# Gyeeta/gyeeta

Measured on NVIDIA H100. Metric: events/sec aggregated, higher is better.
Workload: dtype u64

## Files before the change

### gyeeta_b200/csrc/gysk_device.cuh

```cuda
#pragma once

#include <cstdint>
#include <cuda_runtime.h>

namespace gysk {

struct HistCell { unsigned long long count; long long sum; };
static constexpr int HIST_CELLS = 16;
static constexpr int HIST_MAX_CELL = 15;

struct alignas(16) TblEntry { unsigned long long key; uint32_t slot1; uint32_t pad; };
static constexpr uint32_t SLOT_INVALID = 0xFFFFFFFFu;

struct Centroid { double mean; unsigned long long weight; };
static constexpr int TD_CAP = 256;

struct alignas(16) Bin { unsigned long long cw; unsigned long long us; };
static constexpr int NBINS = 848;
static constexpr int BIN_CNT_BITS = 27;
static constexpr unsigned long long BIN_CNT_MASK = (1ull << BIN_CNT_BITS) - 1;
static constexpr int HOT_ROW_BINS = 1024, HOT_ROW_WORDS = 2 * HOT_ROW_BINS;
static_assert(NBINS <= HOT_ROW_BINS, "a row holds every bin");
__host__ __device__ __forceinline__ uint32_t hot_word(uint32_t bin) { return ((bin & 31u) << 5) | (bin >> 5); }

struct alignas(8) SlotAux { unsigned long long act_cur, act_last, err_cur, err_last; uint32_t rtt_cur, rtt_last; };

struct alignas(16) SlotBatch { uint32_t minv, maxv, touched, hot; };
struct alignas(8) SlotState { uint8_t state, issue, issue_bits, high_bits; uint32_t nconn_active; };

struct TdHead { unsigned long long total; double minv, maxv; uint32_t n; uint32_t pad; };

struct IdTable
{
	TblEntry	*ent;
	uint32_t	mask;
	uint32_t	max_slots;
	uint32_t	*count;
	unsigned long long *slot_id;
	uint32_t	*slot_host;
	int32_t		*free_n;
	uint32_t	*free_slots;
	unsigned long long *insert_fail;
};
static constexpr unsigned long long KEY_TOMBSTONE = ~0ull;

enum { CTR_IN = 0, CTR_DROPPED, CTR_RESP, CTR_TCP, CTR_TASK, CTR_FOREIGN, CTR_NKEYS, CTR_INSERT_FAIL, CTR_NTOUCHED ,
	CTR_NLONG , CTR_NEVICT, CTR_EVICTED_TOTAL,
	CTR_NHOT , CTR_NHOT_NEXT , CTR_NWINDOW ,
	CTR_NHOSTS , CTR_MAX };

static constexpr uint32_t JHASH_GOLDEN = 0x9e3779b9u;
static constexpr uint32_t GY_SEED = 0xceedfeadu;
static constexpr uint32_t FLOW_SEED_A = GY_SEED;
static constexpr uint32_t FLOW_SEED_B = GY_SEED ^ 0x5bd1e995u;

__host__ __device__ __forceinline__ uint32_t jhash_2words(uint32_t a, uint32_t b, uint32_t initval)
{
	uint32_t c = initval;

	a += JHASH_GOLDEN; b += JHASH_GOLDEN;
	a -= b; a -= c; a ^= (c >> 13);
	b -= c; b -= a; b ^= (a << 8);
	c -= a; c -= b; c ^= (b >> 13);
	a -= b; a -= c; a ^= (c >> 12);
	b -= c; b -= a; b ^= (a << 16);
	c -= a; c -= b; c ^= (b >> 5);
	a -= b; a -= c; a ^= (c >> 3);
	b -= c; b -= a; b ^= (a << 10);
	c -= a; c -= b; c ^= (b >> 15);
	return c;
}

__host__ __device__ __forceinline__ uint32_t uint64_hash(unsigned long long key)
{
	return jhash_2words((uint32_t)(key & 0xFFFFFFFFu), (uint32_t)(key >> 32), GY_SEED);
}

__host__ __device__ __forceinline__ uint32_t table_hash(unsigned long long key)
{
	return (uint32_t)((key * 0x9E3779B97F4A7C15ull) >> 32);
}

__host__ __device__ __forceinline__ void flow_hashes(unsigned long long key, uint32_t &h1, uint32_t &h2)
{
	const uint32_t lo = (uint32_t)key, hi = (uint32_t)(key >> 32);
	h1 = jhash_2words(lo, hi, FLOW_SEED_A);
	h2 = jhash_2words(lo, hi, FLOW_SEED_B);
}

__host__ __device__ __forceinline__ uint32_t cms_index2(uint32_t h1, uint32_t h2, uint32_t row, uint32_t wmask)
{
	return (h1 + row * (h2 | 1u)) & wmask;
}

__host__ __device__ __forceinline__ uint32_t cms_index(unsigned long long key, uint32_t row, uint32_t wmask)
{
	uint32_t h1, h2;
	flow_hashes(key, h1, h2);
	return cms_index2(h1, h2, row, wmask);
}

__host__ __device__ __forceinline__ unsigned long long cms_increment(uint32_t bytes)
{
	return 1ull | ((unsigned long long)(bytes >> 10) << 32);
}

__device__ __forceinline__ void hll_idx_rank2(uint32_t h1, uint32_t h2, uint32_t p, uint32_t &idx, uint32_t &rank)
{
	const unsigned long long h = ((unsigned long long)h2 << 32) | h1;
	const unsigned long long w = h << p;

	idx = (uint32_t)(h >> (64 - p));
	rank = w ? (uint32_t)__clzll((long long)w) + 1u : (64u - p + 1u);
}

static constexpr int TD_CODE_BITS = 10;
__host__ __device__ __forceinline__ uint32_t td_code(uint32_t v)
{
#ifdef __CUDA_ARCH__
	if (v < 32u) return v;
	const uint32_t sh = (31u - (uint32_t)__clz((int)v)) - 5u;
#else
	if (v < 32u) return v;
	const uint32_t sh = (31u - (uint32_t)__builtin_clz(v)) - 5u;
#endif
	return ((sh + 1u) << 5) | ((v >> sh) & 31u);
}
__host__ __device__ __forceinline__ uint32_t td_code_lo(uint32_t c) { return c < 32u ? c : ((32u | (c & 31u)) << ((c >> 5) - 1u)); }
__host__ __device__ __forceinline__ uint32_t td_code_hi(uint32_t c) { return c < 32u ? c : (((32u | (c & 31u)) + 1u) << ((c >> 5) - 1u)) - 1u; }

// ... 178 lines not shown
```

### gyeeta_b200/csrc/gysk_kernels.cu

```cuda
#include "gysk_kernels.cuh"
#include "gysk_state.cuh"
#include "gysk_summary.cuh"

#include <cfloat>
#include <climits>
#include <cmath>
#include <algorithm>
#include <type_traits>
#include <cstdlib>
#include <cstring>

namespace gysk {

static constexpr int KEY_GROUP_SHIFT = 30;
static constexpr int KEY_SLOT_SHIFT = KEY_GROUP_SHIFT + TD_CODE_BITS;
__device__ __forceinline__ uint32_t key_usec(unsigned long long k) { return (uint32_t)k & 0x3FFFFFFFu; }
__device__ __forceinline__ uint32_t key_slot(unsigned long long k) { return (uint32_t)(k >> KEY_SLOT_SHIFT); }
__device__ __forceinline__ uint32_t key_bin(unsigned long long k) { return (uint32_t)(k >> KEY_GROUP_SHIFT) & ((1u << TD_CODE_BITS) - 1u); }

static constexpr int KEY_DIGIT_MAX = 8;
static constexpr int KEY_SLOT_BITS_MAX = 24;
static constexpr int KEY_PASSES_MAX = (TD_CODE_BITS + KEY_SLOT_BITS_MAX + KEY_DIGIT_MAX - 1) / KEY_DIGIT_MAX;
static_assert(KEY_PASSES_MAX <= OS_MAX_PASSES, "a RESP plan fits a SortPlan");
struct SortPlan { int np; int shift[OS_MAX_PASSES]; int bits[OS_MAX_PASSES]; };
// ... 823 lines not shown
	}
#pragma unroll
	for (int t = 0; t < LS_V; ++t) {
		const bool act = tail[t];
		if (!__any_sync(0xffffffffu, act)) continue;
		const uint32_t did = act ? pd[t] : (0x80000000u | (uint32_t)lane);
		const unsigned long long v = act ? ps[t] : 0ull;
		uint32_t cnt = act ? pc[t] : 0u, rem = act ? prem[t] : 0u;
		const uint32_t m = __match_any_sync(0xffffffffu, did);
		unsigned long long gsum = v;
		const uint32_t maxcnt = __reduce_max_sync(0xffffffffu, (uint32_t)__popc(m));
		uint32_t rest = m & ~(1u << lane);
		const uint32_t cnt0 = cnt, rem0 = rem;
		for (uint32_t u = 1; u < maxcnt; ++u) {
			const int src = rest ? (__ffs(rest) - 1) : lane;
			const unsigned long long ov = __shfl_sync(0xffffffffu, v, src);
			const uint32_t oc = __shfl_sync(0xffffffffu, cnt0, src), orr = __shfl_sync(0xffffffffu, rem0, src);
			if (rest) { gsum += ov; cnt += oc; rem += orr; rest &= rest - 1; }
		}
		if (act && (m & ((1u << lane) - 1u)) == 0) red_bin(did, (unsigned long long)cnt | ((unsigned long long)rem << BIN_CNT_BITS), gsum);
	}
}

__global__ void __launch_bounds__(256) long_sum_kernel(const unsigned long long *__restrict__ keys, const unsigned long long *__restrict__ d_n,
		const BatchSeg *__restrict__ segs, const unsigned long long *__restrict__ nlong, unsigned long long *__restrict__ rows)
{
	if (*nlong == 0) return;
	const uint64_t n = *d_n;
	const uint64_t nchunks = (n + 127) >> 7;
	const int lane = threadIdx.x & 31;
	const uint64_t gw = ((uint64_t)blockIdx.x * blockDim.x + threadIdx.x) >> 5, nwarps = ((uint64_t)gridDim.x * blockDim.x) >> 5;
	for (uint64_t c0 = gw * 32; c0 < nchunks; c0 += nwarps * 32) {
		const uint64_t c = c0 + lane;
		uint32_t sf = 0, sl = 0, rf = 0, rl = 0;
		if (c < nchunks) {
			const uint64_t f = c << 7, l = f + 127 < n ? f + 127 : n - 1;
			sf = key_slot(keys[f]); sl = key_slot(keys[l]);
			rf = segs[sf].row1; rl = segs[sl].row1;
		}
		for (uint32_t todo = __ballot_sync(0xffffffffu, (rf | rl) != 0); todo; todo &= todo - 1) {
			const int src = __ffs(todo) - 1;
			long_sum_chunk(keys, n, (c0 + (uint64_t)src) << 7, __shfl_sync(0xffffffffu, sf, src), __shfl_sync(0xffffffffu, rf, src),
					__shfl_sync(0xffffffffu, sl, src), __shfl_sync(0xffffffffu, rl, src), rows);
		}
	}
}

static constexpr int TD_WARPS = 3;
static constexpr int TD_SMEM_N = 540;

__global__ void __launch_bounds__(TD_WARPS * 32, TD_MERGE_CTAS_PER_SM) bins_merge_kernel(DevState st, const unsigned long long *__restrict__ keys,
		const uint32_t *__restrict__ touched, const unsigned long long *__restrict__ ntouched_p, const uint32_t *__restrict__ long_slot,
		const unsigned long long *__restrict__ nlong_p, unsigned long long *__restrict__ batch_rows, const BatchSeg *__restrict__ segs,
		Centroid *__restrict__ items_scratch , TdWorkBig *__restrict__ big_scratch , int exp)
{
	__shared__ TdWorkT<TD_SMEM_N> work[TD_WARPS];
	__shared__ uint32_t hcnt[TD_WARPS][16], hsum_lo[TD_WARPS][16], hsum_hi[TD_WARPS][16];
	__shared__ uint8_t bk_tab[NBINS / 8];
	const int lane = threadIdx.x & 31, wid = threadIdx.x >> 5;
	const uint32_t gw = blockIdx.x * TD_WARPS + wid, nwarps = gridDim.x * TD_WARPS;

	Centroid *items = items_scratch + (size_t)gw * NBINS;
	const uint32_t ntouched = (uint32_t)*ntouched_p, nlong = (uint32_t)*nlong_p;

	for (uint32_t g = threadIdx.x; g < (uint32_t)NBINS / 8; g += blockDim.x) {
		constexpr uint32_t thr[13] = {1, 10, 30, 60, 100, 150, 200, 300, 450, 700, 1000, 3000, 15000};
		auto bucket = [&](uint32_t bin) {
			uint32_t bk = bin >= 1u;
			for (int q = 2; q < 15; ++q) bk += bin >= td_code((thr[q - 2] + 1u) * 1000u) + (uint32_t)q;
			return bk;
		};
		const uint32_t b0 = bucket(g * 8);
		uint32_t off = 8;
		for (uint32_t o = 7; o >= 1; --o) if (bucket(g * 8 + o) != b0) off = o;
		bk_tab[g] = (uint8_t)(b0 | (off << 4));
	}
	__syncthreads();

	const uint32_t nhot = st.hot_rows ? (uint32_t)st.counters[CTR_NHOT] : 0u;
	const uint32_t nrow = nhot + nlong, total = nrow + ntouched;
	const uint32_t lt = (1u << lane) - 1u;
	auto slot_of = [&](uint32_t t) { return t < nhot ? st.hot_slot[t] : (t < nrow ? long_slot[t - nhot] : touched[t - nrow]); };
	uint32_t nslot = gw < total ? slot_of(gw) : 0u;
	for (uint32_t t = gw; t < total; t += nwarps) {
		const uint32_t slot = nslot;
		const bool has_next = t + nwarps < total;
		nslot = has_next ? slot_of(t + nwarps) : 0u;
		const SlotBatch sb = st.slot_batch[slot];
		BatchSeg seg {0u, 0u, 0u, 0u};
		if (t >= nrow) seg = segs[slot];
		uint2 nseg = make_uint2(0u, 0u);
		if (has_next) {
			prefetch_l2(st.td_cent + (size_t)nslot * TD_CAP + lane * (TD_CAP / 32));
			if (lane == 0) prefetch_l2(st.slot_batch + nslot);
			else if (lane == 1) prefetch_l2(st.td_head + nslot);
			if (t + nwarps >= nrow) { const BatchSeg ns = segs[nslot]; nseg = make_uint2(ns.key0, ns.end); }
		}
		if (t < nhot && sb.minv == 0xFFFFFFFFu) continue;
		if (lane < 16) { hcnt[wid][lane] = 0; hsum_lo[wid][lane] = 0; hsum_hi[wid][lane] = 0; }
		__syncwarp();
		const uint32_t na = st.td_head[slot].n;
		TdWorkT<TD_SMEM_N> &W = work[wid];
		auto take_bin = [&](uint32_t j, unsigned long long cw, unsigned long long us, uint32_t bin, bool staged) {
			const unsigned long long cnt = cw & BIN_CNT_MASK, rem = cw >> BIN_CNT_BITS;
			const double mean = __ddiv_rn((double)us, (double)cnt);
			if (staged) { W.src[na + j] = mean; W.nxt[j] = (uint16_t)cnt; }
			else { Centroid c; c.mean = mean; c.weight = cnt; items[j] = c; }
			const uint32_t e = bk_tab[bin >> 3], bk = (e & 15u) + ((bin & 7u) >= (e >> 4) ? 1u : 0u);
			atomicAdd(&hcnt[wid][bk], (uint32_t)cnt);
			const unsigned long long ms = (us - rem) / 1000ull;
			const uint32_t mlo = (uint32_t)ms, mhi = (uint32_t)(ms >> 32);
			const uint32_t old = atomicAdd(&hsum_lo[wid][bk], mlo);
			const uint32_t up = mhi + (old + mlo < old ? 1u : 0u);
			if (up) atomicAdd(&hsum_hi[wid][bk], up);
		};
		uint32_t nitems = 0, nsamples, binmax = 0;
		bool staged = false;
		if (t >= nrow) {
			nsamples = seg.end - seg.key0;
			constexpr int RAW_BIN_SHIFT = 54;
			static_assert(BIN_CNT_BITS + 10 + 14 <= RAW_BIN_SHIFT && LONG_SEG <= (1 << 14), "cw of a short segment's bin below the bin bits");
			const uint32_t room = (uint32_t)TD_SMEM_N - na;
			unsigned long long *raw_us = reinterpret_cast<unsigned long long *>(W.src + na), *raw_cw = W.pref;
			ulonglong2 *raw = reinterpret_cast<ulonglong2 *>(items);
			auto load8 = [&](uint32_t b0, unsigned long long (&k)[8]) {
				const uint32_t i0 = b0 + (uint32_t)lane * 8u;
				if (i0 >= seg.key0 && i0 + 8u <= seg.end) {
#pragma unroll
					for (int q = 0; q < 4; ++q) {
						const ulonglong2 v = *reinterpret_cast<const ulonglong2 *>(keys + i0 + 2 * q);
						k[2 * q] = v.x; k[2 * q + 1] = v.y;
					}
				}
				else {
#pragma unroll
					for (int u = 0; u < 8; ++u) k[u] = i0 + u >= seg.key0 && i0 + u < seg.end ? keys[i0 + u] : ~0ull;
				}
			};
			auto rem_of = [](uint32_t v) { return v - (v / 1000u) * 1000u; };
			uint32_t pbin = ~0u, ccnt = 0, crem = 0;
			unsigned long long cus = 0;
			const uint32_t a0 = seg.key0 & ~1u;
			unsigned long long kk[8], nk[8];
			load8(a0, kk);
			for (uint32_t b0 = a0; b0 < seg.end; b0 += 256) {
				if (b0 + 256u < seg.end) load8(b0 + 256u, nk);
				else {
#pragma unroll
					for (int u = 0; u < 8; ++u) nk[u] = ~0ull;
				}
				uint32_t bin[8];
#pragma unroll
				for (int u = 0; u < 8; ++u) bin[u] = kk[u] == ~0ull ? ~0u : key_bin(kk[u]);
				const uint32_t nfirst = __shfl_sync(0xffffffffu, nk[0] == ~0ull ? ~0u : key_bin(nk[0]), 0);
				uint32_t prevb = __shfl_up_sync(0xffffffffu, bin[7], 1), nextb = __shfl_down_sync(0xffffffffu, bin[0], 1);
				if (lane == 0) prevb = pbin;
				if (lane == 31) nextb = nfirst;
				uint32_t hc = 0, tc = 0, tr = 0;
				unsigned long long tu = 0;
#pragma unroll
				for (int u = 0; u < 8; ++u) {
					const bool valid = bin[u] != ~0u;
					if (valid && bin[u] != (u ? bin[u - 1] : prevb)) { ++hc; tc = 0; tr = 0; tu = 0; }
					const uint32_t v = key_usec(kk[u]);
					if (valid) { ++tc; tr += rem_of(v); tu += v; }
				}
				const unsigned long long X = tu | ((unsigned long long)hc << 40);
				const uint32_t Y = tr | (tc << 18);
				unsigned long long xi = X;
				uint32_t yi = Y;
#pragma unroll
				for (int off = 1; off < 32; off <<= 1) {
					const unsigned long long x = __shfl_up_sync(0xffffffffu, xi, off);
					const uint32_t y = __shfl_up_sync(0xffffffffu, yi, off);
					if (lane >= off) { xi += x; yi += y; }
				}
				const uint32_t hm = __ballot_sync(0xffffffffu, hc != 0);
				const uint32_t upto = hm & (0xFFFFFFFFu >> (31 - lane));
				const int h = upto ? 31 - __clz((int)upto) : 0;
				const unsigned long long xs = xi - __shfl_sync(0xffffffffu, xi - X, h);
				const uint32_t ys = yi - __shfl_sync(0xffffffffu, yi - Y, h);
				unsigned long long su = xs & ((1ull << 40) - 1u);
				uint32_t sc = ys >> 18, sr = ys & 0x3FFFFu;
				if (!upto) { su += cus; sc += ccnt; sr += crem; }
				unsigned long long ru = __shfl_up_sync(0xffffffffu, su, 1);
				uint32_t rc = __shfl_up_sync(0xffffffffu, sc, 1), rr = __shfl_up_sync(0xffffffffu, sr, 1);
				if (lane == 0) { ru = cus; rc = ccnt; rr = crem; }
				uint32_t j = nitems + (uint32_t)(xi >> 40) - hc - 1u;
#pragma unroll
				for (int u = 0; u < 8; ++u) {
					const bool valid = bin[u] != ~0u;
					if (valid && bin[u] != (u ? bin[u - 1] : prevb)) { ++j; rc = 0; rr = 0; ru = 0; }
					const uint32_t v = key_usec(kk[u]);
					if (valid) { ++rc; rr += rem_of(v); ru += v; }
					if (valid && bin[u] != (u < 7 ? bin[u + 1] : nextb)) {
						const unsigned long long cwb = (unsigned long long)rc | ((unsigned long long)rr << BIN_CNT_BITS) |
								((unsigned long long)bin[u] << RAW_BIN_SHIFT);
						if (j < room) { raw_us[j] = ru; raw_cw[j] = cwb; }
						else raw[j] = make_ulonglong2(ru, cwb);
						binmax = max(binmax, rc);
					}
				}
				cus = __shfl_sync(0xffffffffu, su, 31); ccnt = __shfl_sync(0xffffffffu, sc, 31); crem = __shfl_sync(0xffffffffu, sr, 31);
				pbin = __shfl_sync(0xffffffffu, bin[7], 31);
				nitems += (uint32_t)(__shfl_sync(0xffffffffu, xi, 31) >> 40);
#pragma unroll
				for (int u = 0; u < 8; ++u) kk[u] = nk[u];
			}
			staged = na + nitems <= (uint32_t)TD_SMEM_N;
			__syncwarp();
			for (uint32_t j = lane; j < nitems; j += 32) {
				const ulonglong2 r = j < room ? make_ulonglong2(raw_us[j], raw_cw[j]) : raw[j];
				take_bin(j, r.y & ((1ull << RAW_BIN_SHIFT) - 1u), r.x, (uint32_t)(r.y >> RAW_BIN_SHIFT), staged);
			}
		}
		else {
			unsigned long long *row = t < nhot ? st.hot_rows + (size_t)t * HOT_ROW_WORDS : batch_rows + (size_t)(t - nhot) * HOT_ROW_WORDS;
			uint32_t mine = 0;
			for (uint32_t b0 = 0; b0 < (uint32_t)NBINS; b0 += 32) {
				const uint32_t bin = b0 + lane;
				const uint32_t i0 = hot_word(bin), i1 = i0 + (uint32_t)HOT_ROW_BINS;
				ulonglong2 v = make_ulonglong2(0ull, 0ull);
				if (bin < (uint32_t)NBINS) { v.x = __ldcg(row + i0); v.y = __ldcg(row + i1); }
				const bool ne = (v.x & BIN_CNT_MASK) != 0;
				const uint32_t m = __ballot_sync(0xffffffffu, ne);
				if (ne) {
					take_bin(nitems + __popc(m & lt), v.x, v.y, bin, false);
					row[i0] = 0ull; row[i1] = 0ull;
					mine += (uint32_t)(v.x & BIN_CNT_MASK);
					binmax = max(binmax, (uint32_t)(v.x & BIN_CNT_MASK));
				}
				nitems += __popc(m);
			}
			nsamples = __reduce_add_sync(0xffffffffu, mine);
		}
		if (has_next && t + nwarps >= nrow) {
			const uint32_t l0 = nseg.x >> 4, l1 = (nseg.y - 1u) >> 4;
			if (l0 + lane <= l1) prefetch_l2(keys + (size_t)(l0 + lane) * 16);
		}
		binmax = __reduce_max_sync(0xffffffffu, binmax);
		__syncwarp();
		if (lane < HIST_MAX_CELL) {
			if (hcnt[wid][lane]) {
				HistCell *c = st.hist_cur + (size_t)slot * HIST_CELLS + lane;
				c->count += hcnt[wid][lane]; c->sum += (long long)(((unsigned long long)hsum_hi[wid][lane] << 32) | hsum_lo[wid][lane]);
			}
		}
		else if (lane == HIST_MAX_CELL) {
			HistCell *c = st.hist_cur + (size_t)slot * HIST_CELLS + HIST_MAX_CELL;
			const long long mx = (long long)(sb.maxv / 1000u);
			if (mx > c->sum) c->sum = mx;
			uint32_t hot = sb.hot;
			if (!hot && st.hot_rows && nsamples >= st.hot_min && nsamples <= st.hot_max && binmax <= st.hot_bin_max) {
				const unsigned long long h = atomicAdd(st.counters + CTR_NHOT_NEXT, 1ull);
				if (h < (unsigned long long)st.hot_cap) { st.hot_slot[h] = slot; hot = (uint32_t)h + 1u; }
				else atomicAdd(st.counters + CTR_NHOT_NEXT, ~0ull);
			}
			st.slot_batch[slot] = SlotBatch {0xFFFFFFFFu, 0u, 0u, hot};
		}
		__syncwarp();
		if (exp & 256) continue;

		TdHead head = st.td_head[slot];
		Centroid *cent = st.td_cent + (size_t)slot * TD_CAP;
		uint32_t nout;
		if (staged) nout = warp_merge_compress_staged(W, cent, na, nitems, cent, st.td);
		else if (na + nitems <= (uint32_t)TD_SMEM_N) nout = warp_merge_compress(W, cent, na, items, nitems, cent, st.td);
		else nout = warp_merge_compress(big_scratch[gw], cent, na, items, nitems, cent, st.td);
		if (lane == 0) {
			head.n = nout;
			head.total += nsamples;
			if ((double)sb.minv < head.minv) head.minv = (double)sb.minv;
			if ((double)sb.maxv > head.maxv) head.maxv = (double)sb.maxv;
			st.td_head[slot] = head;
		}
		__syncwarp();
	}
}

__global__ void flush_kernel(DevState st, uint32_t nslots, uint32_t tsec, uint32_t idle_secs)
{
	const uint64_t i = (uint64_t)blockIdx.x * blockDim.x + threadIdx.x;
	const bool valid = i < (uint64_t)nslots * HIST_CELLS;
	const int cell = (int)(i & (HIST_CELLS - 1));
	HistCell c {0, 0};
	unsigned long long cc = 0;
	const uint32_t slot = (uint32_t)(i >> 4);

	if (valid) {
		c = st.hist_cur[i];
		if (cell == HIST_MAX_CELL) cc = st.conn_cur[slot];
	}
	bool auxact = false;
	if (valid && cell == HIST_MAX_CELL) { const SlotAux a0 = st.slot_aux[slot]; auxact = (a0.act_cur | a0.err_cur) != 0; }
	const uint32_t bal = __ballot_sync(0xffffffffu, valid && (cell == HIST_MAX_CELL ? (cc != 0 || auxact) : c.count != 0));
	const bool active = ((bal >> (threadIdx.x & 16)) & 0xFFFFu) != 0;
	if (!valid) return;

	st.bm_last[i] = st.bm_cur[i]; st.bm_cur[i] = 0;
	st.hist_last[i] = c;
	HistCell &r0 = st.levels.row(0, st.levels.cur[0], slot)[cell], &r1 = st.levels.row(1, st.levels.cur[1], slot)[cell];
	if (cell == HIST_MAX_CELL) {
		if (c.sum > r0.sum) r0.sum = c.sum;
		if (c.sum > r1.sum) r1.sum = c.sum;
	}
	else {
		r0.count += c.count; r0.sum += c.sum;
		r1.count += c.count; r1.sum += c.sum;
	}
	if (cell == HIST_MAX_CELL) {
		if (c.sum > st.hist_all[i].sum) st.hist_all[i].sum = c.sum;
		st.hist_cur[i].count = 0; st.hist_cur[i].sum = LLONG_MIN;
		st.conn_last[slot] = cc;
		st.conn_all_cnt[slot] += (uint32_t)cc;
		st.conn_all_kb[slot] += cc >> 32;
		st.conn_cur[slot] = 0;
		{
			SlotAux a = st.slot_aux[slot];
			a.act_last = a.act_cur; a.act_cur = 0; a.err_last = a.err_cur; a.err_cur = 0; a.rtt_last = a.rtt_cur; a.rtt_cur = 0;
// ... 521 lines not shown
	if (!(exp & 4)) { launch_drain_pass<false>(st, tmp, rr, n_events, exp, dev, s); launches++; }
	if (!(exp & 8)) { launch_drain_pass<true>(st, tmp, rr, n_events, exp, dev, s); launches++; }
	return launches;
}

static void os_set_attrs(int dev)
{
	static bool attr_set[MAX_DEVICES] = {};
	if (attr_set[dev]) return;
	cudaFuncSetAttribute(os_pass_kernel<6>, cudaFuncAttributeMaxDynamicSharedMemorySize, (int)sizeof(OneSweepSharedT<6>));
	cudaFuncSetAttribute(os_pass_kernel<7>, cudaFuncAttributeMaxDynamicSharedMemorySize, (int)sizeof(OneSweepSharedT<7>));
	cudaFuncSetAttribute(os_pass_kernel<8>, cudaFuncAttributeMaxDynamicSharedMemorySize, (int)sizeof(OneSweepSharedT<8>));
	cudaFuncSetAttribute(os_pass_kernel<9>, cudaFuncAttributeMaxDynamicSharedMemorySize, (int)sizeof(OneSweepSharedT<9>));
	cudaFuncSetAttribute(os_hist_kernel<8, 257>, cudaFuncAttributeMaxDynamicSharedMemorySize, OS_MAX_PASSES * 8 * 257 * (int)sizeof(uint32_t));
	cudaFuncSetAttribute(os_hist_kernel<4, 513>, cudaFuncAttributeMaxDynamicSharedMemorySize, OS_MAX_PASSES * 4 * 513 * (int)sizeof(uint32_t));
	attr_set[dev] = true;
}

static uint32_t next_epoch(const SortTemp &tmp, uint32_t max_tiles, cudaStream_t s)
{
	uint32_t e = ++*tmp.epoch;
	if (e == 0) {
		cudaMemsetAsync(tmp.tile_status, 0, (size_t)max_tiles * RADIX_MAX * sizeof(unsigned long long), s);
		e = ++*tmp.epoch;
	}
	return e;
}

static int launch_sort_passes(const SortPlan &P, const SortTemp &tmp, const unsigned long long *d_n, uint32_t ntiles, int *which, cudaStream_t s)
{
	unsigned long long *bufs[2] = { tmp.keys_a, tmp.keys_b };
	const uint32_t grid = std::min<uint32_t>(ntiles, (uint32_t)sm_count(current_device()) * 4u);
	int w = 0;

	for (int p = 0; p < P.np; ++p, w ^= 1) {
		const uint32_t epoch = next_epoch(tmp, tmp.max_tiles, s);
		auto pass = [&](auto kernel, size_t smem) {
			kernel<<<grid, OS_THREADS, smem, s>>>(bufs[w], bufs[w ^ 1], d_n, P.shift[p], P.bits[p], tmp.os_ghist + p * RADIX_MAX, tmp.tile_status,
					tmp.os_ghist + OS_GHIST_TICKETS + p, epoch);
		};
		if (P.bits[p] > 8) pass(os_pass_kernel<9>, sizeof(OneSweepSharedT<9>));
		else if (P.bits[p] == 8) pass(os_pass_kernel<8>, sizeof(OneSweepSharedT<8>));
		else if (P.bits[p] == 7) pass(os_pass_kernel<7>, sizeof(OneSweepSharedT<7>));
		else pass(os_pass_kernel<6>, sizeof(OneSweepSharedT<6>));
	}
	*which = w;
	return P.np;
}

int launch_radix_sort(const SortTemp &tmp, const unsigned long long *d_n, uint64_t n_max, int lo, int hi, int *which, cudaStream_t s)
{
	SortPlan P;

	*which = 0;
	if (!n_max) return 0;
	if (plain_sort_plan(lo, hi, P) || n_max >= (1ull << 30)) return -1;
	bool any9 = false;
	for (int p = 0; p < P.np; ++p) any9 |= P.bits[p] > 8;
	const int copies = any9 ? 4 : 8, stride = (any9 ? 512 : 256) + 1;
	const int dev = current_device();
	os_set_attrs(dev);

	cudaMemsetAsync(tmp.os_ghist, 0, OS_GHIST_WORDS * sizeof(uint32_t), s);
	const uint32_t hgrid = std::min<uint32_t>(div_up(n_max, 512 * 2 * 4), (uint32_t)sm_count(dev) * 3);
	if (any9) os_hist_kernel<4, 513><<<hgrid, 512, (size_t)P.np * copies * stride * sizeof(uint32_t), s>>>(tmp.keys_a, d_n, P, tmp.os_ghist);
	else os_hist_kernel<8, 257><<<hgrid, 512, (size_t)P.np * copies * stride * sizeof(uint32_t), s>>>(tmp.keys_a, d_n, P, tmp.os_ghist);
	return 1 + launch_sort_passes(P, tmp, d_n, div_up(n_max, SORT_TILE), which, s);
}

int launch_batch_merge(const DevState &st, const SortTemp &tmp, uint64_t n_events, uint32_t max_svcs, cudaStream_t s)
{
	if (!n_events) return 0;
	unsigned long long *d_nkeys = st.counters + CTR_NKEYS, *d_ntouched = st.counters + CTR_NTOUCHED;
	const int dev = current_device();
	const int nsm = sm_count(dev);
	os_set_attrs(dev);

	SortPlan plan {};
	if (key_sort_plan(max_svcs, plan) < 0) return -1;
	int which = 0;
	const int launches = launch_sort_passes(plan, tmp, d_nkeys, div_up(n_events, SORT_TILE), &which, s);
	const unsigned long long *src = which ? tmp.keys_b : tmp.keys_a;

	static_assert(CTR_NLONG == CTR_NTOUCHED + 1, "one memset clears both segment counters");
	unsigned long long *d_nlong = st.counters + CTR_NLONG;
	BatchSeg *segs = reinterpret_cast<BatchSeg *>(tmp.segs);
	cudaMemsetAsync(d_ntouched, 0, 2 * sizeof(unsigned long long), s);
	segs_mark_kernel<<<div_up(n_events, SG_THREADS * SG_V), SG_THREADS, 0, s>>>(src, d_nkeys, segs, tmp.touched, d_ntouched, tmp.long_slot, d_nlong);
	long_sum_kernel<<<nsm * 8, 256, 0, s>>>(src, d_nkeys, segs, d_nlong, tmp.batch_rows);
	const int merge_ctas = std::min(nsm, TD_MERGE_MAX_SMS) * TD_MERGE_CTAS_PER_SM;
	bins_merge_kernel<<<merge_ctas, TD_WARPS * 32, 0, s>>>(st, src, tmp.touched, d_ntouched, tmp.long_slot, d_nlong, tmp.batch_rows, segs,
			tmp.items_scratch, tmp.big_scratch, exp_ablate());
	return launches + 3;
}

__global__ void topn_score_kernel(DevState st, uint32_t nslots, int metric, int host_filter, unsigned long long *__restrict__ keys,
		unsigned long long *d_n)
{
	const uint32_t slot = blockIdx.x * blockDim.x + threadIdx.x;
	if (slot == 0) *d_n = nslots;
	if (slot >= nslots) return;
	unsigned long long score = 0;

	if (host_filter < 0 || st.slot_host[slot] == (uint32_t)host_filter) {
		if (metric == GYSK_TOPN_QPS) {
			for (int b = 0; b < HIST_MAX_CELL; ++b) score += st.hist_last[(size_t)slot * HIST_CELLS + b].count;
		}
		else if (metric == GYSK_TOPN_CONNS) score = (uint32_t)st.conn_last[slot];
		else if (metric == GYSK_TOPN_ISSUE) {
			const SlotState ss = st.slot_state[slot];
			score = ss.state > GYSK_STATE_OK && ss.state <= GYSK_STATE_DOWN ? ss.state : 0;
		}
		else if (metric == GYSK_TOPN_ACTIVE) score = (uint32_t)st.slot_aux[slot].act_last;
		else score = st.conn_last[slot] >> 32;
	}
	if (score > 0xFFFFFFFFull) score = 0xFFFFFFFFull;
	keys[slot] = (score << 32) | slot;
}

__global__ void topn_task_score_kernel(DevState st, uint32_t ntasks, int metric, unsigned long long *__restrict__ keys, unsigned long long *d_n)
{
	const uint32_t slot = blockIdx.x * blockDim.x + threadIdx.x;
	if (slot == 0) *d_n = ntasks;
	if (slot >= ntasks) return;
	unsigned long long score = st.task_slot_id[slot] ? (unsigned long long)st.task_last[(size_t)slot * 3 + metric].sum : 0ull;
	if ((long long)score < 0) score = 0;
	if (score > 0xFFFFFFFFull) score = 0xFFFFFFFFull;
	keys[slot] = (score << 32) | slot;
}

__global__ void topn_pick_kernel(const unsigned long long *__restrict__ slot_id, const uint32_t *__restrict__ slot_host,
		const unsigned long long *__restrict__ sorted, uint32_t nslots, uint32_t want, gysk_topn_entry *__restrict__ out,
		unsigned long long *__restrict__ slots)
{
	const uint32_t i = threadIdx.x;
	if (i >= want) return;
	gysk_topn_entry o; o.glob_id = 0; o.score = 0; o.host_idx = 0; o.pad = 0;
	uint32_t slot = 0;
	if (i < nslots) {
		const unsigned long long k = sorted[nslots - 1 - i];
		slot = (uint32_t)k;
		o.glob_id = slot_id[slot]; o.score = k >> 32; o.host_idx = slot_host ? slot_host[slot] : 0u;
	}
	out[i] = o;
	if (slots) slots[i] = slot;
}

int launch_topn_pick(const SortTemp &tmp, const unsigned long long *d_n, uint32_t nkeys, const unsigned long long *ids, const uint32_t *hosts,
		uint32_t want, gysk_topn_entry *d_out, cudaStream_t s, unsigned long long *d_slots)
{
	int which = 0;
	const int sorted = launch_radix_sort(tmp, d_n, nkeys, 32, 64, &which, s);
	if (sorted < 0) return sorted;
	topn_pick_kernel<<<1, 64, 0, s>>>(ids, hosts, which ? tmp.keys_b : tmp.keys_a, nkeys, want, d_out, d_slots);
	return sorted + 1;
}

int launch_topn(const DevState &st, const SortTemp &tmp, uint32_t nslots, int is_task, int metric, int host_filter, uint32_t want,
		gysk_topn_entry *d_out, cudaStream_t s, unsigned long long *d_slots)
{
	if (!nslots) return 0;
	unsigned long long *d_n = st.counters + CTR_NKEYS;
	if (is_task) topn_task_score_kernel<<<div_up(nslots, 256), 256, 0, s>>>(st, nslots, metric, tmp.keys_a, d_n);
	else topn_score_kernel<<<div_up(nslots, 256), 256, 0, s>>>(st, nslots, metric, host_filter, tmp.keys_a, d_n);
	const int picked = launch_topn_pick(tmp, d_n, nslots, is_task ? st.task_slot_id : st.slot_id, is_task ? st.task_slot_host : st.slot_host,
			want, d_out, s, d_slots);
	return picked < 0 ? picked : 1 + picked;
}

__global__ void task_flush_kernel(DevState st, uint32_t max_tasks)
// ... 129 lines not shown
```

### gyeeta_b200/csrc/gysk_tdigest.cuh

```cuda
#pragma once

#include "gysk_device.cuh"

namespace gysk {

struct TdParams { const double *qtab; uint32_t delta; uint32_t pad; };

template <int NMAX_>
struct TdWorkT
{
	static constexpr int NMAX = NMAX_;
	double			mean[NMAX];
	unsigned long long	pref[NMAX + 1];
	uint16_t		bounds[TD_CAP + 2];
	uint16_t		nxt[NMAX];
	double			src[NMAX];
};
using TdWork = TdWorkT<2 * TD_CAP>;
using TdWorkBig = TdWorkT<1120>;
struct TdScratch : TdWork
{
	Centroid		newc[TD_CAP];
};

template <bool B_STAGED, typename Work>
__device__ __forceinline__ uint32_t td_merge_compress(Work &S, const Centroid *a, uint32_t na, const Centroid *b, uint32_t nb,
		Centroid *out, const TdParams &P)
{
	const int lane = threadIdx.x & 31;
	const uint32_t nm = na + nb;

	double *am = S.src, *bm = S.src + na;
	for (uint32_t j0 = 0; j0 < na; j0 += 32 * 4) {
		double v[4];
#pragma unroll
		for (int q = 0; q < 4; ++q) { const uint32_t j = j0 + q * 32 + lane; v[q] = j < na ? a[j].mean : 0.0; }
#pragma unroll
		for (int q = 0; q < 4; ++q) { const uint32_t j = j0 + q * 32 + lane; if (j < na) am[j] = v[q]; }
	}
	if (!B_STAGED) for (uint32_t j = lane; j < nb; j += 32) bm[j] = b[j].mean;
	__syncwarp();
	const uint32_t per = (nm + 31u) >> 5;
	const uint32_t d0 = lane * per < nm ? lane * per : nm, d1 = d0 + per < nm ? d0 + per : nm;
	unsigned long long tot = 0;
	if (d0 < d1) {
		uint32_t lo = d0 > nb ? d0 - nb : 0u, hi = d0 < na ? d0 : na;
		while (lo < hi) { const uint32_t mid = (lo + hi) >> 1; if (am[mid] <= bm[d0 - 1u - mid]) lo = mid + 1; else hi = mid; }
		uint32_t i = lo, k = d0 - lo;
		double av = i < na ? am[i] : 0.0, bv = k < nb ? bm[k] : 0.0;
		constexpr unsigned long long FROM_A = 1ull << 63;
		for (uint32_t pos = d0; pos < d1; ++pos) {
			const bool ta = i < na && (k >= nb || av <= bv);
			S.mean[pos] = ta ? av : bv;
			if (B_STAGED) S.pref[pos + 1] = ta ? (FROM_A | i) : (unsigned long long)S.nxt[k];
			else S.nxt[pos] = (uint16_t)(ta ? i : (0x8000u | k));
			if (ta) { ++i; av = i < na ? am[i] : 0.0; }
			else { ++k; bv = k < nb ? bm[k] : 0.0; }
		}
		for (uint32_t p0 = d0; p0 < d1; p0 += 4) {
			unsigned long long w[4];
#pragma unroll
			for (int q = 0; q < 4; ++q) {
				const uint32_t pos = p0 + q < d1 ? p0 + q : d1 - 1u;
				if (B_STAGED) { const unsigned long long f = S.pref[pos + 1]; w[q] = (f & FROM_A) ? a[(uint32_t)f].weight : f; }
				else { const uint32_t from = S.nxt[pos]; w[q] = (from & 0x8000u) ? b[from & 0x7FFFu].weight : a[from].weight; }
			}
#pragma unroll
			for (int q = 0; q < 4; ++q) if (p0 + q < d1) { S.pref[p0 + q + 1] = w[q]; tot += w[q]; }
		}
	}
	{
		unsigned long long incl = tot;
#pragma unroll
		for (int off = 1; off < 32; off <<= 1) {
			const unsigned long long tt = __shfl_up_sync(0xffffffffu, incl, off);
			if (lane >= off) incl += tt;
		}
		unsigned long long run = incl - tot;
		for (uint32_t pos = d0; pos < d1; ++pos) { run += S.pref[pos + 1]; S.pref[pos + 1] = run; }
		if (lane == 0) S.pref[0] = 0;
	}
	__syncwarp();
	auto ckey = [&S](uint32_t i) { const unsigned long long p = S.pref[i]; return p + ((S.pref[i + 1] - p) >> 1); };

	uint32_t nout = 0;
	if (nm) {
		const unsigned long long Wt = S.pref[nm];
		const double W = (double)Wt;
		const uint32_t cj = (P.delta + 32u) >> 5;
		uint32_t lo = 0;
		for (uint32_t j = lane * cj, jn = 0; jn < cj && j <= P.delta; ++j, ++jn) {
			const unsigned long long T = j == P.delta ? Wt : (unsigned long long)__dmul_rn(__ldg(P.qtab + j), W);
			uint32_t steps = jn ? 0u : 8u;
			while (steps < 8u && lo < nm && ckey(lo) < T) { ++lo; ++steps; }
			if (steps == 8u) {
				uint32_t hi = nm;
				while (lo < hi) { const uint32_t mid = (lo + hi) >> 1; if (ckey(mid) < T) lo = mid + 1; else hi = mid; }
			}
			S.nxt[j] = (uint16_t)lo;
		}
		__syncwarp();
		for (uint32_t j0 = 0; j0 < P.delta; j0 += 32) {
			const uint32_t j = j0 + lane;
			const bool ne = j < P.delta && S.nxt[j + 1] > S.nxt[j];
			const uint32_t m = __ballot_sync(0xffffffffu, ne);
			if (ne) S.bounds[nout + __popc(m & ((1u << lane) - 1u))] = S.nxt[j];
			nout += __popc(m);
		}
		if (lane == 0) S.bounds[nout] = (uint16_t)nm;
		__syncwarp();
	}

	for (uint32_t c = lane; c < nout; c += 32) {
		double csum = 0.0;
		const uint32_t lo = S.bounds[c], hi = S.bounds[c + 1];
		for (uint32_t i = lo; i < hi; ++i) {
			csum = __dadd_rn(csum, __dmul_rn(S.mean[i], (double)(S.pref[i + 1] - S.pref[i])));
		}
		const unsigned long long cw = S.pref[hi] - S.pref[lo];
		Centroid o; o.mean = __ddiv_rn(csum, (double)cw); o.weight = cw;
		out[c] = o;
	}
	__syncwarp();
	return nout;
}

template <typename Work>
__device__ __forceinline__ uint32_t warp_merge_compress(Work &S, const Centroid *a, uint32_t na, const Centroid *b, uint32_t nb,
		Centroid *out, const TdParams &P)
{
	return td_merge_compress<false>(S, a, na, b, nb, out, P);
}

template <typename Work>
__device__ __forceinline__ uint32_t warp_merge_compress_staged(Work &S, const Centroid *a, uint32_t na, uint32_t nb, Centroid *out,
		const TdParams &P)
{
	return td_merge_compress<true>(S, a, na, nullptr, nb, out, P);
}

}
```

Measured before the change: 12.21 billion.

## Use dynamic work cursor in bins merge and restructure t-digest merge weight gathering

The bins merge kernel now hands out slots from a global atomic work counter instead of a fixed warp stride, which is meant to balance load across warps when slots differ in cost. A new counter is added to the enum and cleared by the existing memset. The t-digest merge now loads centroids as 16-byte vectors held in registers and scatters weights by recorded output positions, instead of indirect gathers from global memory. It also precomputes the quantile thresholds into registers before the boundary search. The cost is one atomic per slot per warp and a larger register footprint.

```diff
diff --git a/gyeeta_b200/csrc/gysk_device.cuh b/gyeeta_b200/csrc/gysk_device.cuh
--- a/gyeeta_b200/csrc/gysk_device.cuh
+++ b/gyeeta_b200/csrc/gysk_device.cuh
@@ -45,7 +45,7 @@
 static constexpr unsigned long long KEY_TOMBSTONE = ~0ull;
 
 enum { CTR_IN = 0, CTR_DROPPED, CTR_RESP, CTR_TCP, CTR_TASK, CTR_FOREIGN, CTR_NKEYS, CTR_INSERT_FAIL, CTR_NTOUCHED ,
-	CTR_NLONG , CTR_NEVICT, CTR_EVICTED_TOTAL,
+	CTR_NLONG , CTR_MERGE_NEXT , CTR_NEVICT, CTR_EVICTED_TOTAL,
 	CTR_NHOT , CTR_NHOT_NEXT , CTR_NWINDOW ,
 	CTR_NHOSTS , CTR_MAX };
 
diff --git a/gyeeta_b200/csrc/gysk_kernels.cu b/gyeeta_b200/csrc/gysk_kernels.cu
--- a/gyeeta_b200/csrc/gysk_kernels.cu
+++ b/gyeeta_b200/csrc/gysk_kernels.cu
@@ -929,10 +929,13 @@
 	const uint32_t lt = (1u << lane) - 1u;
 	auto slot_of = [&](uint32_t t) { return t < nhot ? st.hot_slot[t] : (t < nrow ? long_slot[t - nhot] : touched[t - nrow]); };
 	uint32_t nslot = gw < total ? slot_of(gw) : 0u;
-	for (uint32_t t = gw; t < total; t += nwarps) {
+	uint32_t tn = 0;
+	for (uint32_t t = gw; t < total; t = tn) {
 		const uint32_t slot = nslot;
-		const bool has_next = t + nwarps < total;
-		nslot = has_next ? slot_of(t + nwarps) : 0u;
+		if (lane == 0) tn = nwarps + (uint32_t)atomicAdd(st.counters + CTR_MERGE_NEXT, 1ull);
+		tn = __shfl_sync(0xffffffffu, tn, 0);
+		const bool has_next = tn < total;
+		nslot = has_next ? slot_of(tn) : 0u;
 		const SlotBatch sb = st.slot_batch[slot];
 		BatchSeg seg {0u, 0u, 0u, 0u};
 		if (t >= nrow) seg = segs[slot];
@@ -941,7 +944,7 @@
 			prefetch_l2(st.td_cent + (size_t)nslot * TD_CAP + lane * (TD_CAP / 32));
 			if (lane == 0) prefetch_l2(st.slot_batch + nslot);
 			else if (lane == 1) prefetch_l2(st.td_head + nslot);
-			if (t + nwarps >= nrow) { const BatchSeg ns = segs[nslot]; nseg = make_uint2(ns.key0, ns.end); }
+			if (tn >= nrow) { const BatchSeg ns = segs[nslot]; nseg = make_uint2(ns.key0, ns.end); }
 		}
 		if (t < nhot && sb.minv == 0xFFFFFFFFu) continue;
 		if (lane < 16) { hcnt[wid][lane] = 0; hsum_lo[wid][lane] = 0; hsum_hi[wid][lane] = 0; }
@@ -1081,7 +1084,7 @@
 			}
 			nsamples = __reduce_add_sync(0xffffffffu, mine);
 		}
-		if (has_next && t + nwarps >= nrow) {
+		if (has_next && tn >= nrow) {
 			const uint32_t l0 = nseg.x >> 4, l1 = (nseg.y - 1u) >> 4;
 			if (l0 + lane <= l1) prefetch_l2(keys + (size_t)(l0 + lane) * 16);
 		}
@@ -1769,10 +1772,11 @@
 	const int launches = launch_sort_passes(plan, tmp, d_nkeys, div_up(n_events, SORT_TILE), &which, s);
 	const unsigned long long *src = which ? tmp.keys_b : tmp.keys_a;
 
-	static_assert(CTR_NLONG == CTR_NTOUCHED + 1, "one memset clears both segment counters");
+	static_assert(CTR_NLONG == CTR_NTOUCHED + 1 && CTR_MERGE_NEXT == CTR_NTOUCHED + 2,
+			"one memset clears both segment counters and bins_merge_kernel's work cursor");
 	unsigned long long *d_nlong = st.counters + CTR_NLONG;
 	BatchSeg *segs = reinterpret_cast<BatchSeg *>(tmp.segs);
-	cudaMemsetAsync(d_ntouched, 0, 2 * sizeof(unsigned long long), s);
+	cudaMemsetAsync(d_ntouched, 0, 3 * sizeof(unsigned long long), s);
 	segs_mark_kernel<<<div_up(n_events, SG_THREADS * SG_V), SG_THREADS, 0, s>>>(src, d_nkeys, segs, tmp.touched, d_ntouched, tmp.long_slot, d_nlong);
 	long_sum_kernel<<<nsm * 8, 256, 0, s>>>(src, d_nkeys, segs, d_nlong, tmp.batch_rows);
 	const int merge_ctas = std::min(nsm, TD_MERGE_MAX_SMS) * TD_MERGE_CTAS_PER_SM;
diff --git a/gyeeta_b200/csrc/gysk_tdigest.cuh b/gyeeta_b200/csrc/gysk_tdigest.cuh
--- a/gyeeta_b200/csrc/gysk_tdigest.cuh
+++ b/gyeeta_b200/csrc/gysk_tdigest.cuh
@@ -20,7 +20,7 @@
 using TdWorkBig = TdWorkT<1120>;
 struct TdScratch : TdWork
 {
-	Centroid		newc[TD_CAP];
+	alignas(16) Centroid	newc[TD_CAP];
 };
 
 template <bool B_STAGED, typename Work>
@@ -30,45 +30,59 @@
 	const int lane = threadIdx.x & 31;
 	const uint32_t nm = na + nb;
 
+	constexpr int AQ = TD_CAP / 32;
 	double *am = S.src, *bm = S.src + na;
-	for (uint32_t j0 = 0; j0 < na; j0 += 32 * 4) {
-		double v[4];
+	unsigned long long aw[AQ];
+	{
+		ulonglong2 v[AQ];
 #pragma unroll
-		for (int q = 0; q < 4; ++q) { const uint32_t j = j0 + q * 32 + lane; v[q] = j < na ? a[j].mean : 0.0; }
+		for (int q = 0; q < AQ; ++q) {
+			const uint32_t j = (uint32_t)(lane + 32 * q);
+			v[q] = j < na ? reinterpret_cast<const ulonglong2 *>(a)[j] : make_ulonglong2(0ull, 0ull);
+		}
 #pragma unroll
-		for (int q = 0; q < 4; ++q) { const uint32_t j = j0 + q * 32 + lane; if (j < na) am[j] = v[q]; }
+		for (int q = 0; q < AQ; ++q) {
+			const uint32_t j = (uint32_t)(lane + 32 * q);
+			if (j < na) am[j] = __longlong_as_double((long long)v[q].x);
+			aw[q] = v[q].y;
+		}
 	}
 	if (!B_STAGED) for (uint32_t j = lane; j < nb; j += 32) bm[j] = b[j].mean;
 	__syncwarp();
 	const uint32_t per = (nm + 31u) >> 5;
 	const uint32_t d0 = lane * per < nm ? lane * per : nm, d1 = d0 + per < nm ? d0 + per : nm;
-	unsigned long long tot = 0;
 	if (d0 < d1) {
 		uint32_t lo = d0 > nb ? d0 - nb : 0u, hi = d0 < na ? d0 : na;
 		while (lo < hi) { const uint32_t mid = (lo + hi) >> 1; if (am[mid] <= bm[d0 - 1u - mid]) lo = mid + 1; else hi = mid; }
 		uint32_t i = lo, k = d0 - lo;
+		const uint32_t k0 = k;
 		double av = i < na ? am[i] : 0.0, bv = k < nb ? bm[k] : 0.0;
-		constexpr unsigned long long FROM_A = 1ull << 63;
 		for (uint32_t pos = d0; pos < d1; ++pos) {
 			const bool ta = i < na && (k >= nb || av <= bv);
 			S.mean[pos] = ta ? av : bv;
-			if (B_STAGED) S.pref[pos + 1] = ta ? (FROM_A | i) : (unsigned long long)S.nxt[k];
-			else S.nxt[pos] = (uint16_t)(ta ? i : (0x8000u | k));
+			if (ta) S.bounds[i] = (uint16_t)pos;
+			else if (B_STAGED) S.pref[pos + 1] = S.nxt[k];
+			else S.nxt[k] = (uint16_t)pos;
 			if (ta) { ++i; av = i < na ? am[i] : 0.0; }
 			else { ++k; bv = k < nb ? bm[k] : 0.0; }
 		}
-		for (uint32_t p0 = d0; p0 < d1; p0 += 4) {
+		if (!B_STAGED) for (uint32_t kq = k0; kq < k; kq += 4) {
 			unsigned long long w[4];
 #pragma unroll
-			for (int q = 0; q < 4; ++q) {
-				const uint32_t pos = p0 + q < d1 ? p0 + q : d1 - 1u;
-				if (B_STAGED) { const unsigned long long f = S.pref[pos + 1]; w[q] = (f & FROM_A) ? a[(uint32_t)f].weight : f; }
-				else { const uint32_t from = S.nxt[pos]; w[q] = (from & 0x8000u) ? b[from & 0x7FFFu].weight : a[from].weight; }
-			}
+			for (int q = 0; q < 4; ++q) w[q] = b[kq + q < k ? kq + q : k - 1u].weight;
 #pragma unroll
-			for (int q = 0; q < 4; ++q) if (p0 + q < d1) { S.pref[p0 + q + 1] = w[q]; tot += w[q]; }
+			for (int q = 0; q < 4; ++q) if (kq + q < k) S.pref[S.nxt[kq + q] + 1u] = w[q];
 		}
 	}
+	__syncwarp();
+#pragma unroll
+	for (int q = 0; q < AQ; ++q) {
+		const uint32_t j = (uint32_t)(lane + 32 * q);
+		if (j < na) S.pref[S.bounds[j] + 1u] = aw[q];
+	}
+	__syncwarp();
+	unsigned long long tot = 0;
+	for (uint32_t pos = d0; pos < d1; ++pos) tot += S.pref[pos + 1];
 	{
 		unsigned long long incl = tot;
 #pragma unroll
@@ -87,15 +101,26 @@
 	if (nm) {
 		const unsigned long long Wt = S.pref[nm];
 		const double W = (double)Wt;
+		constexpr int CJ = (TD_CAP + 32) / 32;
 		const uint32_t cj = (P.delta + 32u) >> 5;
+		const uint32_t jl = lane * cj;
+		double qj[CJ];
+#pragma unroll
+		for (int jn = 0; jn < CJ; ++jn) qj[jn] = (uint32_t)jn < cj && jl + jn < P.delta ? __ldg(P.qtab + jl + jn) : 0.0;
+		unsigned long long T[CJ];
+#pragma unroll
+		for (int jn = 0; jn < CJ; ++jn) T[jn] = jl + jn == P.delta ? Wt : (unsigned long long)__dmul_rn(qj[jn], W);
 		uint32_t lo = 0;
-		for (uint32_t j = lane * cj, jn = 0; jn < cj && j <= P.delta; ++j, ++jn) {
-			const unsigned long long T = j == P.delta ? Wt : (unsigned long long)__dmul_rn(__ldg(P.qtab + j), W);
+#pragma unroll 1
+		for (uint32_t jn = 0, j = jl; jn < cj && j <= P.delta; ++jn, ++j) {
+			const unsigned long long Tj = T[0];
+#pragma unroll
+			for (int q = 0; q + 1 < CJ; ++q) T[q] = T[q + 1];
 			uint32_t steps = jn ? 0u : 8u;
-			while (steps < 8u && lo < nm && ckey(lo) < T) { ++lo; ++steps; }
+			while (steps < 8u && lo < nm && ckey(lo) < Tj) { ++lo; ++steps; }
 			if (steps == 8u) {
 				uint32_t hi = nm;
-				while (lo < hi) { const uint32_t mid = (lo + hi) >> 1; if (ckey(mid) < T) lo = mid + 1; else hi = mid; }
+				while (lo < hi) { const uint32_t mid = (lo + hi) >> 1; if (ckey(mid) < Tj) lo = mid + 1; else hi = mid; }
 			}
 			S.nxt[j] = (uint16_t)lo;
 		}
```

New measurement: 12.49 billion, median of 6. No clear change (+2.3%).
